# matteo-bastico/MI-Seg

Hardware: AMD Instinct MI355X
Metric: 96^3 patches/sec fwd+bwd, C-Swin-UNETR fs=48 6-class (higher is better)
Workload: dtype bf16; 1 GPU; configs[1]: C-Swin-UNETR feature_size=48 heads=(3,6,12,24) instance_cond, 96^3 patch, 6 classes, batch 1 per GPU, fwd+bwd (+ gradient all-reduce at N>1); global_batch=1

## Files before the change

### include/miseg_hip.h

```cpp
#ifndef MISEG_HIP_H
#define MISEG_HIP_H
#include <stddef.h>
#include <stdint.h>

#ifdef __cplusplus
extern "C" {
#endif

typedef void* miseg_stream_t;

enum { MISEG_F32 = 0, MISEG_BF16 = 1 };
enum { MISEG_OK = 0, MISEG_E_BADARG = -1, MISEG_E_UNSUPPORTED = -2, MISEG_E_LAUNCH = -3 };
enum { MISEG_ACT_NONE = 0, MISEG_ACT_LEAKY = 1, MISEG_ACT_GELU = 2, MISEG_ACT_PRELU = 3 };
#define MISEG_MAX_STYLES 4

#define MISEG_ABI_VERSION 16
int miseg_abi_version(void);
const char* miseg_last_error(void);
int miseg_device_arch(char* buf, size_t n);

size_t miseg_instnorm_stat_bytes(int B, int C);
typedef struct {
  const void* x; int64_t ldx;
  int B, S, C, dtype;
// ... 199 lines not shown
typedef struct {
  const void* qkv; int64_t ldq; void* out; int64_t ldo;
  const float* qkv_bias;
  const float* bias_table;
  float* lse;
  int B, D, H, W, C, heads, dtype;
  int wd, wh, ww, sd, sh, sw, tw;
  float scale;
  float drop_p; uint64_t drop_seed, drop_stream; const uint64_t* drop_step_dev;
} miseg_winattn_params;
int miseg_winattn_fwd(const miseg_winattn_params* p, miseg_stream_t stream);
int miseg_winattn_on_matrix_cores(const miseg_winattn_params* p);

typedef struct {
  miseg_winattn_params f;
  const void* dout; int64_t lddo;
  void* dqkv; int64_t lddq;
  float* dqkv_bias;
  float* dbias_table;
} miseg_winattn_bwd_params;
int miseg_winattn_bwd(const miseg_winattn_bwd_params* p, miseg_stream_t stream);
int miseg_winattn_bwd_on_matrix_cores(const miseg_winattn_bwd_params* p);

typedef struct { const void* a; int64_t lda; const void* b; int64_t ldb; void* y; int64_t ldy; int64_t rows; int C, dtype; } miseg_add_params;
int miseg_add(const miseg_add_params* p, miseg_stream_t stream);
typedef struct { uint32_t struct_size; const void* a; int64_t lda; const void* x; int64_t ldx; void* y; int64_t ldy; const float* coef; int B, S, C, dtype; } miseg_affine2_params;
int miseg_affine2(const miseg_affine2_params* p, miseg_stream_t stream);

typedef struct { const void* src; int64_t lds; int sdtype; void* dst; int64_t ldd; int ddtype; int64_t rows; int C; } miseg_copy2d_params;
int miseg_copy2d(const miseg_copy2d_params* p, miseg_stream_t stream);

typedef struct { const float* src; void* dst; int R, C, dtype, transpose; } miseg_cast_params;
int miseg_cast_matrix(const miseg_cast_params* p, miseg_stream_t stream);

typedef struct {
  const float* src; void* dst;
  int32_t R, C, transpose, inner, outer, tile0;
} miseg_cast_desc;
int miseg_param_cast_batch(const miseg_cast_desc* descs_dev, int ndesc, int total_tiles, int dtype, const int64_t* params_version, int64_t* state,
                           miseg_stream_t stream);

typedef struct { const void* x; int64_t ldx; void* y; int64_t ldy; int64_t rows; int C, dtype; } miseg_gelu_fwd_params;
int miseg_gelu_fwd(const miseg_gelu_fwd_params* p, miseg_stream_t stream);
typedef struct { const void* dy; int64_t lddy; const void* x; int64_t ldx; void* dx; int64_t lddx; int64_t rows; int C, dtype; } miseg_gelu_bwd_params;
int miseg_gelu_bwd(const miseg_gelu_bwd_params* p, miseg_stream_t stream);

// ... 331 lines not shown
```

### mi-seg_amd/csrc/attention.hip

```cpp
#include "common.h"

namespace miseg {

struct WinGeom {
  int B, D, H, W, C, heads, hd;
  int wd, wh, ww, sd, sh, sw, tw;
  int Dp, Hp, Wp, nwd, nwh, nww, n;
  float scale;
};

__device__ __forceinline__ void token_info(const WinGeom& g, int win, int t, int& row, int& label, int& code) {
  int wi = win;
  const int wx = wi % g.nww; wi /= g.nww;
  const int wy = wi % g.nwh; wi /= g.nwh;
  const int wz = wi % g.nwd;
  const int b = wi / g.nwd;
  const int tz = t / (g.wh * g.ww), ty = (t / g.ww) % g.wh, tx = t % g.ww;
  const int pz = wz * g.wd + tz, py = wy * g.wh + ty, px = wx * g.ww + tx;
  int z = pz + g.sd; if (z >= g.Dp) z -= g.Dp;
  int y = py + g.sh; if (y >= g.Hp) y -= g.Hp;
  int x = px + g.sw; if (x >= g.Wp) x -= g.Wp;
  row = (z < g.D && y < g.H && x < g.W) ? ((b * g.D + z) * g.H + y) * g.W + x : -1;
  const int rz = g.sd ? (pz < g.Dp - g.wd ? 0 : (pz < g.Dp - g.sd ? 1 : 2)) : 0;
  const int ry = g.sh ? (py < g.Hp - g.wh ? 0 : (py < g.Hp - g.sh ? 1 : 2)) : 0;
// ... 331 lines not shown
  bf16x8 f;
#pragma unroll
  for (int j = 0; j < 8; ++j) f[j] = (bf16)0.f;
  if (r < 16) {
    const bf16* p = base + r * ATT_VT_LD + t0 + 16 * s + 4 * h;
    const bf16x4 lo = *reinterpret_cast<const bf16x4*>(p);
    const bf16x4 hi = *reinterpret_cast<const bf16x4*>(p + 8);
    f = bf16x8{lo[0], lo[1], lo[2], lo[3], hi[0], hi[1], hi[2], hi[3]};
  }
  return f;
}

__device__ __forceinline__ void att_load16v(const bf16* p, bool vec, float* dst) {
  if (vec) {
    const bf16x8 a = *reinterpret_cast<const bf16x8*>(p), b = *reinterpret_cast<const bf16x8*>(p + 8);
#pragma unroll
    for (int d = 0; d < 8; ++d) { dst[d] = to_f32(a[d]); dst[8 + d] = to_f32(b[d]); }
  } else {
#pragma unroll
    for (int d = 0; d < 16; ++d) dst[d] = to_f32(p[d]);
  }
}

__device__ __forceinline__ void att_unit(int heads, int& win, int& head) {
  const int nb = gridDim.x, xcd = blockIdx.x & 7, q = nb >> 3, r = nb & 7;
  const int unit = xcd * q + (xcd < r ? xcd : r) + (blockIdx.x >> 3);
  win = unit / heads;
  head = unit - win * heads;
}

template <bool MASK, int NW = 4, bool DROP = false>
__global__ void __launch_bounds__(NW * 64) winattn_fwd_mfma_kernel(const bf16* __restrict__ qkv, int64_t ldq, bf16* __restrict__ out, int64_t ldo,
                                                               const float* __restrict__ qkv_bias, const float* __restrict__ bias_table,
                                                               float* __restrict__ lse_out, WinGeom g, int tsize, bool vec, AttnDrop dr) {
  extern __shared__ __attribute__((aligned(16))) char smem[];
  bf16* Qs = reinterpret_cast<bf16*>(smem);
  bf16* Ks = Qs + ATT_NP * 16;
  bf16* Vt = Ks + ATT_NP * 16;
  int* kofs = reinterpret_cast<int*>(Vt + 16 * ATT_VT_LD);
  int* klab = kofs + ATT_NP;
  int* rowq = klab + ATT_NP;
  float* table = reinterpret_cast<float*>(rowq + ATT_NP);
  int win, head;
  att_unit(g.heads, win, head);
  const int tid = threadIdx.x;
  const int n = g.n, C = g.C, ntiles = (n + 31) / 32;
  for (int t = tid; t < ntiles * 32; t += NW * 64) {
    int row = -1, label = 0, code = 0;
    float q[16], k[16], v[16];
#pragma unroll
    for (int d = 0; d < 16; ++d) q[d] = k[d] = v[d] = 0.f;
    if (t < n) {
      token_info(g, win, t, row, label, code);
      if (row >= 0) {
        const bf16* p = qkv + (int64_t)row * ldq + head * 16;
        att_load16v(p, vec, q);
        att_load16v(p + C, vec, k);
        att_load16v(p + 2 * C, vec, v);
      } else if (qkv_bias) {
#pragma unroll
        for (int d = 0; d < 16; ++d) { q[d] = qkv_bias[head * 16 + d]; k[d] = qkv_bias[C + head * 16 + d]; v[d] = qkv_bias[2 * C + head * 16 + d]; }
      }
    }
    const float qs = g.scale * ATT_LOG2E;
#pragma unroll
    for (int d = 0; d < 16; ++d) q[d] *= qs;
    *reinterpret_cast<bf16x8*>(Qs + t * 16) = cvt8(q);
    *reinterpret_cast<bf16x8*>(Qs + t * 16 + 8) = cvt8(q + 8);
    *reinterpret_cast<bf16x8*>(Ks + t * 16) = cvt8(k);
    *reinterpret_cast<bf16x8*>(Ks + t * 16 + 8) = cvt8(k + 8);
#pragma unroll
    for (int d = 0; d < 16; ++d) Vt[d * ATT_VT_LD + t] = (bf16)v[d];
    kofs[t] = code * 4;
    klab[t] = label;
    rowq[t] = row;
  }
  for (int i = tid; i < tsize; i += NW * 64) table[i] = bias_table[(int64_t)i * g.heads + head] * ATT_LOG2E;
  __syncthreads();
  const int lane = tid & 63, wave = __builtin_amdgcn_readfirstlane(tid >> 6), r = lane & 31, h = lane >> 5;
  const int tb = 2 * g.tw - 1;
  const int centre = ((g.tw - 1) * tb + (g.tw - 1)) * tb + (g.tw - 1);
  const bool ragged = (n & 31) != 0;
  constexpr float MASKV = -100.f * ATT_LOG2E;
  const uint64_t dk0 = DROP ? dropout_step_key(dr.key, dr.step_dev) : 0ull;
  const int dcg = (n + 3) / 4;
  for (int qt = wave; qt < ntiles; qt += NW) {
    const int qi = qt * 32 + r;
    const int64_t drow = ((int64_t)win * g.heads + head) * n + qi;
    const bf16x8 qf = *reinterpret_cast<const bf16x8*>(Qs + qi * 16 + 8 * h);
    const char* tq = reinterpret_cast<const char*>(table) + kofs[qi] + 4 * centre;
    const int lq = klab[qi];
    float m = -INFINITY, l = 0.f;
    f32x16 acc;
#pragma unroll
    for (int i = 0; i < 16; ++i) acc[i] = 0.f;
    auto key_tile = [&](int kt, auto last_tag) {
      constexpr bool LAST = decltype(last_tag)::value;
      const bf16x8 kf = *reinterpret_cast<const bf16x8*>(Ks + (kt * 32 + r) * 16 + 8 * h);
      f32x16 sacc;
#pragma unroll
      for (int i = 0; i < 16; ++i) sacc[i] = 0.f;
      sacc = __builtin_amdgcn_mfma_f32_32x32x16_bf16(kf, qf, sacc, 0, 0, 0);
      float sv[16];
#pragma unroll
      for (int gq = 0; gq < 4; ++gq) {
        const int k0 = kt * 32 + 8 * gq + 4 * h;
        const int4 ko = *reinterpret_cast<const int4*>(kofs + k0);
        const int kov[4] = {ko.x, ko.y, ko.z, ko.w};
#pragma unroll
// ... 102 lines not shown

template <bool MASK, bool DT , int NW = 4, bool DROP = false>
__global__ void __launch_bounds__(NW * 64, 2) winattn_bwd_mfma_kernel(const bf16* __restrict__ qkv, int64_t ldq, const bf16* __restrict__ out, int64_t ldo,
                                                                  const bf16* __restrict__ dout, int64_t lddo, bf16* __restrict__ dqkv, int64_t lddq,
                                                                  const float* __restrict__ qkv_bias, const float* __restrict__ bias_table,
                                                                  const float* __restrict__ lse_in, float* __restrict__ dqkv_bias,
                                                                  float* __restrict__ dbias_table, WinGeom g, int tsize, bool vec, AttnDrop dr) {
  extern __shared__ __attribute__((aligned(16))) char smem[];
  constexpr int NI = 24 / NW, NTHR = NW * 64;
  float* table = reinterpret_cast<float*>(smem);
  int* dtable = reinterpret_cast<int*>(table + ATT_TMAX);
  float* padb = reinterpret_cast<float*>(dtable + ATT_TMAX);
  unsigned* bound = reinterpret_cast<unsigned*>(padb + 48);
  char* dstile = reinterpret_cast<char*>(padb + 64);
  float* dqpart = reinterpret_cast<float*>(dstile + NW * 16 * ATT_DS_LD);
  int* qcode = reinterpret_cast<int*>(dqpart + 2 * NW * 256);
  int* qlabel = qcode + ATT_NP;
  int* rowq = qlabel + ATT_NP;
  float* nlse = reinterpret_cast<float*>(rowq + ATT_NP);
  float* ndelta = nlse + ATT_NP;
  bf16* Qs = reinterpret_cast<bf16*>(ndelta + ATT_NP);
  bf16* Gs = Qs + ATT_NP * 16;
  bf16* Ks = Gs + ATT_NP * 16;
  int win, head;
  att_unit(g.heads, win, head);
  const int tid = threadIdx.x;
  const int n = g.n, C = g.C, nt16 = (n + 15) / 16;
  if (tid < 52) padb[tid] = 0.f;
  __syncthreads();
  float mg2 = 0.f, mv2 = 0.f, mda = 0.f;
  for (int t = tid; t < nt16 * 16; t += NTHR) {
    int row = -1, label = 0, code = 0;
    float q[16], k[16], go[16];
    float dl = 0.f, ls = INFINITY, g2 = 0.f, v2 = 0.f;
#pragma unroll
    for (int d = 0; d < 16; ++d) q[d] = k[d] = go[d] = 0.f;
    if (t < n) {
      token_info(g, win, t, row, label, code);
      ls = lse_in[((int64_t)win * g.heads + head) * n + t];
      float v[16];
      if (row >= 0) {
        float o[16];
        att_load16(qkv + (int64_t)row * ldq + head * 16, vec, q);
        att_load16(qkv + (int64_t)row * ldq + C + head * 16, vec, k);
        att_load16(qkv + (int64_t)row * ldq + 2 * C + head * 16, vec, v);
        att_load16(dout + (int64_t)row * lddo + head * 16, vec, go);
        att_load16(out + (int64_t)row * ldo + head * 16, vec, o);
#pragma unroll
// ... 280 lines not shown

static bool fwd_takes_mfma(const miseg_winattn_params* p, const WinGeom& g) {
  return p->dtype == MISEG_BF16 && g.hd == 16 && g.n <= ATT_NP && p->bias_table && ((uintptr_t)p->out % 8 == 0) && p->ldo % 4 == 0;
}

extern "C" int miseg_winattn_on_matrix_cores(const miseg_winattn_params* p) {
  WinGeom g;
  if (!p || make_geom(p, &g)) return 0;
  return (fwd_takes_mfma(p, g) || global_attn_takes(p)) ? 1 : 0;
}

static bool bwd_takes_mfma(const miseg_winattn_bwd_params* p, const WinGeom& g) {
  const int tb = 2 * g.tw - 1;
  return p->f.dtype == MISEG_BF16 && g.hd == 16 && g.n <= ATT_NP && p->f.bias_table && tb * tb * tb <= ATT_TMAX && ((uintptr_t)p->dqkv % 8 == 0) && p->lddq % 4 == 0 &&
         ((uintptr_t)p->f.qkv % 8 == 0) && p->f.ldq % 4 == 0;
}

extern "C" int miseg_winattn_bwd_on_matrix_cores(const miseg_winattn_bwd_params* p) {
  WinGeom g;
  if (!p || !p->dout || !p->dqkv || make_geom(&p->f, &g)) return 0;
  return (bwd_takes_mfma(p, g) || global_attn_bwd_takes(p)) ? 1 : 0;
}

extern "C" int miseg_winattn_fwd(const miseg_winattn_params* p, miseg_stream_t s_) {
  hipStream_t s = (hipStream_t)s_;
  MISEG_REQUIRE(p, MISEG_E_BADARG, "winattn_fwd: null params");
  WinGeom g;
  int rc = make_geom(p, &g);
  if (rc) return rc;
  MISEG_REQUIRE(p->drop_p >= 0.f && p->drop_p < 1.f, MISEG_E_BADARG, "winattn_fwd: drop_p = %f must lie in [0, 1)", (double)p->drop_p);
  const AttnDrop dr = attn_drop_args(p);
  if (global_attn_fwd(p, dr, s, &rc)) return rc;
  const int tb = 2 * g.tw - 1, tsize = p->bias_table ? tb * tb * tb : 0;
  const size_t sh = attn_smem_bytes(g.n, g.hd, tsize, false);
  MISEG_REQUIRE(sh <= 160 * 1024, MISEG_E_UNSUPPORTED, "winattn_fwd: %zu bytes of LDS needed", sh);
  dim3 grid(g.B * g.nwd * g.nwh * g.nww, g.heads);
  const int threads = cdiv(g.n, 64) * 64;
  if (fwd_takes_mfma(p, g)) {
    const size_t shm = attn_mfma_fwd_smem(tsize);
    const bool vec = p->ldq % 8 == 0 && (uintptr_t)p->qkv % 16 == 0;
    const bool wide = (int64_t)grid.x * grid.y < 256;
#define FWD_MFMA_D(M, NWV, D)                                                                                                                  \
  MISEG_SET_SMEM((winattn_fwd_mfma_kernel<M, NWV, D>), shm);                    \
  winattn_fwd_mfma_kernel<M, NWV, D><<<grid.x * grid.y, NWV * 64, shm, s>>>((const bf16*)p->qkv, p->ldq, (bf16*)p->out, p->ldo, p->qkv_bias, p->bias_table, \
                                                                 p->lse, g, tsize, vec, dr)
#define FWD_MFMA(M, NWV) do { if (dr.thresh) { FWD_MFMA_D(M, NWV, true); } else { FWD_MFMA_D(M, NWV, false); } } while (0)
    if ((g.sd | g.sh | g.sw) != 0) { if (wide) { FWD_MFMA(true, 11); } else { FWD_MFMA(true, 8); } }
    else { if (wide) { FWD_MFMA(false, 11); } else { FWD_MFMA(false, 8); } }
#undef FWD_MFMA
#undef FWD_MFMA_D
    MISEG_LAUNCH_CHECK("winattn_fwd_mfma");
    return MISEG_OK;
  }
  return dispatch_dtype(p->dtype, [&](auto* tag) -> int {
    typedef typename std::remove_pointer<decltype(tag)>::type T;
    HD_SWITCH(g.hd / 4, {
      MISEG_SET_SMEM((winattn_fwd_kernel<T, HD4>), sh);
      winattn_fwd_kernel<T, HD4><<<grid, threads, sh, s>>>((const T*)p->qkv, p->ldq, (T*)p->out, p->ldo, p->qkv_bias, p->bias_table, p->lse, g, tsize, dr);
    });
    MISEG_LAUNCH_CHECK("winattn_fwd");
    return MISEG_OK;
  });
}

extern "C" int miseg_winattn_bwd(const miseg_winattn_bwd_params* p, miseg_stream_t s_) {
  hipStream_t s = (hipStream_t)s_;
  MISEG_REQUIRE(p && p->dout && p->dqkv, MISEG_E_BADARG, "winattn_bwd: null pointer");
  MISEG_REQUIRE(!p->dbias_table || p->f.bias_table, MISEG_E_BADARG, "winattn_bwd: dbias_table given without a bias_table");
  WinGeom g;
  int rc = make_geom(&p->f, &g);
  if (rc) return rc;
  MISEG_REQUIRE(p->f.drop_p >= 0.f && p->f.drop_p < 1.f, MISEG_E_BADARG, "winattn_bwd: drop_p = %f must lie in [0, 1)", (double)p->f.drop_p);
  const AttnDrop dr = attn_drop_args(&p->f);
  if (global_attn_bwd(p, dr, s, &rc)) return rc;
  const int tb = 2 * g.tw - 1, tsize = p->f.bias_table ? tb * tb * tb : 0;
  const size_t sh = attn_smem_bytes(g.n, g.hd, tsize, true);
  MISEG_REQUIRE(sh <= 160 * 1024, MISEG_E_UNSUPPORTED, "winattn_bwd: %zu bytes of LDS needed", sh);
  dim3 grid(g.B * g.nwd * g.nwh * g.nww, g.heads);
  const int threads = cdiv(g.n, 64) * 64;
  if (bwd_takes_mfma(p, g)) {
    const bool vec = p->f.ldq % 8 == 0 && p->f.ldo % 8 == 0 && p->lddo % 8 == 0 && (uintptr_t)p->f.qkv % 16 == 0 && (uintptr_t)p->f.out % 16 == 0 &&
                     (uintptr_t)p->dout % 16 == 0;
    const bool wide = true;
    const size_t shm = attn_mfma_bwd_smem(tsize, wide ? 8 : 4);
#define BWD_MFMA_X(M, D, NWV, X)                                                                                                                            \
// ... 28 lines not shown
```

### mi-seg_amd/csrc/common.cpp

```cpp
#include "common.h"
#include "../../include/miseg_hip_debug.h"
#include <string.h>

#ifndef MISEG_COMPILED_ARCH
#define MISEG_COMPILED_ARCH "gfx950"
#endif

namespace miseg {
static thread_local char g_err[512] = "";

int set_error(int code, const char* fmt, ...) {
  va_list ap;
  va_start(ap, fmt);
  vsnprintf(g_err, sizeof(g_err), fmt, ap);
  va_end(ap);
  return code;
}
}

extern "C" int miseg_abi_version(void) { return MISEG_ABI_VERSION; }

extern "C" size_t miseg_abi_struct_size(const char* name) {
  if (!name) return 0;
#define MISEG_SZ(T) if (strcmp(name, #T) == 0) return sizeof(T);
  MISEG_SZ(miseg_instnorm_stats_params) MISEG_SZ(miseg_instnorm_apply_params) MISEG_SZ(miseg_instnorm_bwd_params) MISEG_SZ(miseg_instnorm_pair_bwd_params)
  MISEG_SZ(miseg_layernorm_fwd_params) MISEG_SZ(miseg_layernorm_bwd_params) MISEG_SZ(miseg_gemm_params) MISEG_SZ(miseg_tn_reduce_desc) MISEG_SZ(miseg_gemm_tn_desc) MISEG_SZ(miseg_gemm_tn_stream_desc) MISEG_SZ(miseg_gemm_tn_stream_plan)
  MISEG_SZ(miseg_mlp_params) MISEG_SZ(miseg_colsum_params) MISEG_SZ(miseg_colsum_desc) MISEG_SZ(miseg_conv3_params) MISEG_SZ(miseg_pack_conv3_params) MISEG_SZ(miseg_pack_conv3_desc)
  MISEG_SZ(miseg_conv3_wgrad_params) MISEG_SZ(miseg_conv3_plan_info) MISEG_SZ(miseg_conv3_wgrad_plan_info) MISEG_SZ(miseg_winattn_params) MISEG_SZ(miseg_winattn_bwd_params) MISEG_SZ(miseg_add_params) MISEG_SZ(miseg_copy2d_params)
  MISEG_SZ(miseg_cast_params) MISEG_SZ(miseg_cast_desc) MISEG_SZ(miseg_gelu_fwd_params) MISEG_SZ(miseg_gelu_bwd_params) MISEG_SZ(miseg_s2c_params)
  MISEG_SZ(miseg_patch_embed_params) MISEG_SZ(miseg_patch_embed_bwd_params) MISEG_SZ(miseg_conv3_thin_params) MISEG_SZ(miseg_conv3_thin_wgrad_params)
  MISEG_SZ(miseg_resample2_params) MISEG_SZ(miseg_upsample_cat_params) MISEG_SZ(miseg_upsample_cat_bwd_params) MISEG_SZ(miseg_rowbias_params) MISEG_SZ(miseg_prelu_fwd_params) MISEG_SZ(miseg_prelu_bwd_params) MISEG_SZ(miseg_head_params)
  MISEG_SZ(miseg_head_bwd_params) MISEG_SZ(miseg_im2col3_params) MISEG_SZ(miseg_seg_loss_params) MISEG_SZ(miseg_dice_metric_params) MISEG_SZ(miseg_surface_distance_params) MISEG_SZ(miseg_surface_metrics_params) MISEG_SZ(miseg_surface_dice_params) MISEG_SZ(miseg_opt_desc) MISEG_SZ(miseg_opt_pack_map)
  MISEG_SZ(miseg_opt_step_params) MISEG_SZ(miseg_stitch_params) MISEG_SZ(miseg_aug_sample) MISEG_SZ(miseg_augment_params) MISEG_SZ(miseg_resample3d_params) MISEG_SZ(miseg_label_export_params) MISEG_SZ(miseg_keep_largest_params) MISEG_SZ(miseg_fill_holes_params) MISEG_SZ(miseg_dropout_params)
  MISEG_SZ(miseg_affine2_params) MISEG_SZ(miseg_graph_split_info) MISEG_SZ(miseg_norm_ref) MISEG_SZ(miseg_ensemble_params) MISEG_SZ(miseg_aug_affine_sample) MISEG_SZ(miseg_augment_affine_params)
  MISEG_SZ(miseg_net_end_launch) MISEG_SZ(miseg_head_bwd_plan_info)
#undef MISEG_SZ
  return 0;
}
extern "C" const char* miseg_last_error(void) { return miseg::g_err; }
extern "C" int miseg_device_arch(char* buf, size_t n) {
  if (!buf || n == 0) return MISEG_E_BADARG;
  strncpy(buf, MISEG_COMPILED_ARCH, n);
  buf[n - 1] = 0;
  return MISEG_OK;
}

extern "C" int miseg_device_check(int device) {
  hipDeviceProp_t prop;
  if (hipGetDeviceProperties(&prop, device) != hipSuccess) {
    (void)hipGetLastError();
    return miseg::set_error(MISEG_E_BADARG, "device_check: no HIP device %d", device);
// ... 62 lines not shown
```

### mi-seg_amd/hip/lib.py

```python
import ctypes as C
import os

HERE = os.path.dirname(os.path.abspath(__file__))
LIB_PATH = os.environ.get("MISEG_HIP_LIB") or os.path.join(os.path.dirname(HERE), "csrc", "libmiseg_hip.so")

F32, BF16 = 0, 1
ACT_NONE, ACT_LEAKY, ACT_GELU, ACT_PRELU = 0, 1, 2, 3
MAX_STYLES = 4

vp, i64, i32, f32 = C.c_void_p, C.c_int64, C.c_int, C.c_float
fp4 = vp * MAX_STYLES


class _S(C.Structure):
    pass


ABI_VERSION = 16
C_NAMES = {}


def _struct(name, fields, cname=None):
    t = type(name, (C.Structure,), {"_fields_": fields})
    C_NAMES[t] = cname
# ... 40 lines not shown
                                                                                  ("pad_", i32), ("workspace_bytes", i64)])
TN_STREAM_GROUP_CAP = 8
Colsum = _struct("Colsum", cname="miseg_colsum_params", fields=[("x", vp), ("ldx", i64), ("rows", i64), ("C", i32), ("dtype", i32), ("out", vp), ("accumulate", i32)])
Conv3 = _struct("Conv3", cname="miseg_conv3_params", fields=[("x", vp), ("ldx", i64), ("y", vp), ("ldy", i64), ("wpk", vp), ("B", i32), ("D", i32), ("H", i32),
                          ("W", i32), ("Cin", i32), ("Cout", i32), ("dtype", i32), ("workspace", vp), ("res", vp), ("ldres", i64), ("stat", vp), ("background", i32), ("defer_slabs", i32),
                          ("sc_x", vp), ("ld_sc_x", i64), ("sc_w", vp), ("sc_C", i32), ("s2c_out", vp), ("s2c_C", i32),
                          ("fs_w", vp), ("fs_y", vp), ("ld_fs_y", i64), ("fs_stat", vp)])
PackConv3Desc = _struct("PackConv3Desc", cname="miseg_pack_conv3_desc", fields=[("w", vp), ("fwd_pack", vp), ("bwd_pack", vp), ("Cin", i32), ("Cout", i32), ("tile0", i32), ("pad_", i32)])
PackConv3 = _struct("PackConv3", cname="miseg_pack_conv3_params", fields=[("w", vp), ("fwd_pack", vp), ("bwd_pack", vp), ("Cin", i32), ("Cout", i32), ("dtype", i32)])
Conv3Wgrad = _struct("Conv3Wgrad", cname="miseg_conv3_wgrad_params", fields=[("x", vp), ("ldx", i64), ("dy", vp), ("lddy", i64), ("dw", vp), ("B", i32), ("D", i32),
                                    ("H", i32), ("W", i32), ("Cin", i32), ("Cout", i32), ("dtype", i32), ("accumulate", i32),
                                    ("workspace", vp), ("max_workgroups", i32)])
CONV3_GENERIC, CONV3_FWD96, CONV3_FWD_TINY = 0, 1, 2
Conv3Plan = _struct("Conv3Plan", cname="miseg_conv3_plan_info", fields=[("kernel", i32), ("splits", i32), ("workspace_bytes", C.c_size_t), ("res", i32), ("stat", i32),
                                  ("sc", i32), ("s2c", i32), ("fs", i32), ("defer_slabs", i32)])
CONV3_WGRAD_F32, CONV3_WGRAD_NARROW, CONV3_WGRAD_TINY, CONV3_WGRAD_BF16 = 0, 1, 2, 3
Conv3WgradPlan = _struct("Conv3WgradPlan", cname="miseg_conv3_wgrad_plan_info", fields=[("kernel", i32), ("pad_", i32), ("workspace_bytes", C.c_size_t)])
Winattn = _struct("Winattn", cname="miseg_winattn_params", fields=[("qkv", vp), ("ldq", i64), ("out", vp), ("ldo", i64), ("qkv_bias", vp), ("bias_table", vp),
                              ("lse", vp), ("B", i32), ("D", i32), ("H", i32), ("W", i32), ("C", i32), ("heads", i32),
                              ("dtype", i32), ("wd", i32), ("wh", i32), ("ww", i32), ("sd", i32), ("sh", i32), ("sw", i32),
                              ("tw", i32), ("scale", f32), ("drop_p", f32), ("drop_seed", C.c_uint64), ("drop_stream", C.c_uint64), ("drop_step_dev", vp)])
WinattnBwd = _struct("WinattnBwd", cname="miseg_winattn_bwd_params", fields=[("f", Winattn), ("dout", vp), ("lddo", i64), ("dqkv", vp), ("lddq", i64),
                                    ("dqkv_bias", vp), ("dbias_table", vp)])
Add = _struct("Add", cname="miseg_add_params", fields=[("a", vp), ("lda", i64), ("b", vp), ("ldb", i64), ("y", vp), ("ldy", i64), ("rows", i64), ("C", i32), ("dtype", i32)])
GraphSplitInfo = _struct("GraphSplitInfo", cname="miseg_graph_split_info", fields=[("nodes", i32), ("lanes", i32), ("segments", i32), ("crossing_edges", i32),
                                                                                  ("side_streams", i32), ("main_lane_nodes", i32), ("streams_concurrent", i32)])
Affine2 = _struct("Affine2", cname="miseg_affine2_params", fields=[("struct_size", C.c_uint32), ("a", vp), ("lda", i64), ("x", vp), ("ldx", i64), ("y", vp), ("ldy", i64), ("coef", vp),
                                                                  ("B", i32), ("S", i32), ("C", i32), ("dtype", i32)])
Copy2d = _struct("Copy2d", cname="miseg_copy2d_params", fields=[("src", vp), ("lds", i64), ("sdtype", i32), ("dst", vp), ("ldd", i64), ("ddtype", i32), ("rows", i64), ("C", i32)])
CastDesc = _struct("CastDesc", cname="miseg_cast_desc", fields=[("src", vp), ("dst", vp), ("R", i32), ("C", i32), ("transpose", i32), ("inner", i32), ("outer", i32), ("tile0", i32)])
Resample2 = _struct("Resample2", cname="miseg_resample2_params", fields=[("x", vp), ("ldx", i64), ("y", vp), ("ldy", i64), ("B", i32), ("D", i32), ("H", i32), ("W", i32), ("C", i32),
                                  ("dtype", i32), ("dir", i32)])
UpsampleCat = _struct("UpsampleCat", cname="miseg_upsample_cat_params", fields=[("skip", vp), ("ldskip", i64), ("x", vp), ("ldx", i64), ("out", vp), ("ldout", i64),
                                      ("B", i32), ("D", i32), ("H", i32), ("W", i32), ("Cs", i32), ("Cu", i32), ("factor", i32), ("dtype", i32)])
UpsampleCatBwd = _struct("UpsampleCatBwd", cname="miseg_upsample_cat_bwd_params", fields=[("dcat", vp), ("lddcat", i64), ("dx", vp), ("lddx", i64), ("B", i32), ("D", i32),
                                            ("H", i32), ("W", i32), ("C", i32), ("factor", i32), ("dtype", i32)])
Rowbias = _struct("Rowbias", cname="miseg_rowbias_params", fields=[("x", vp), ("ldx", i64), ("bias", vp), ("y", vp), ("ldy", i64), ("rows", i64), ("C", i32), ("dtype", i32)])
PreluFwd = _struct("PreluFwd", cname="miseg_prelu_fwd_params", fields=[("x", vp), ("ldx", i64), ("slope", vp), ("y", vp), ("ldy", i64), ("rows", i64), ("C", i32), ("dtype", i32)])
PreluBwd = _struct("PreluBwd", cname="miseg_prelu_bwd_params", fields=[("dy", vp), ("lddy", i64), ("x", vp), ("ldx", i64), ("slope", vp), ("dx", vp), ("lddx", i64), ("dslope", vp),
                                ("rows", i64), ("C", i32), ("dtype", i32), ("scratch", vp)])
Cast = _struct("Cast", cname="miseg_cast_params", fields=[("src", vp), ("dst", vp), ("R", i32), ("C", i32), ("dtype", i32), ("transpose", i32)])
GeluFwd = _struct("GeluFwd", cname="miseg_gelu_fwd_params", fields=[("x", vp), ("ldx", i64), ("y", vp), ("ldy", i64), ("rows", i64), ("C", i32), ("dtype", i32)])
GeluBwd = _struct("GeluBwd", cname="miseg_gelu_bwd_params", fields=[("dy", vp), ("lddy", i64), ("x", vp), ("ldx", i64), ("dx", vp), ("lddx", i64), ("rows", i64), ("C", i32), ("dtype", i32)])
S2C = _struct("S2C", cname="miseg_s2c_params", fields=[("src", vp), ("lds", i64), ("dst", vp), ("ldd", i64), ("B", i32), ("D", i32), ("H", i32), ("W", i32),
                      ("C", i32), ("dtype", i32), ("offsets", C.c_int8 * 24)])
PatchEmbed = _struct("PatchEmbed", cname="miseg_patch_embed_params", fields=[("x", vp), ("y", vp), ("ldy", i64), ("w", vp), ("bias", vp), ("B", i32), ("Cin", i32), ("D", i32),
# ... 132 lines not shown
    "miseg_colsum": (i32, [C.POINTER(Colsum), vp]),
    "miseg_gemm_tn_splits": (i32, [C.POINTER(Gemm)]),
    "miseg_gemm_tn_fuses_colsum": (i32, [C.POINTER(Gemm)]),
    "miseg_gemm_tn_reduce_batch": (i32, [vp, i32, vp]),
    "miseg_gemm_tn_group": (i32, [vp, i32, i32, vp]),
    "miseg_gemm_tn_stream_group_plan": (i32, [vp, i32, vp]),
    "miseg_gemm_tn_stream_group": (i32, [vp, i32, vp]),
    "miseg_gemm_tn_stream_group_target": (i32, []),
    "miseg_colsum_batch": (i32, [vp, i32, i32, vp]),
    "miseg_conv3_fwd_plan": (i32, [C.POINTER(Conv3), C.POINTER(Conv3Plan)]),
    "miseg_conv3_fwd": (i32, [C.POINTER(Conv3), vp]),
    "miseg_pack_conv3_elems": (C.c_size_t, [i32, i32, i32, i32]),
    "miseg_pack_conv3_tiles": (i32, [i32, i32, i32]),
    "miseg_pack_conv3_weight": (i32, [C.POINTER(PackConv3), vp]),
    "miseg_pack_conv3_batch": (i32, [vp, i32, i32, i32, vp, vp, vp]),
    "miseg_conv3_wgrad_plan": (i32, [C.POINTER(Conv3Wgrad), C.POINTER(Conv3WgradPlan)]),
    "miseg_conv3_wgrad": (i32, [C.POINTER(Conv3Wgrad), vp]),
    "miseg_conv3_wgrad_group_workspace_bytes": (C.c_size_t, [C.POINTER(Conv3Wgrad), i32]),
    "miseg_conv3_wgrad_group": (i32, [C.POINTER(Conv3Wgrad), i32, vp, vp]),
    "miseg_winattn_fwd": (i32, [C.POINTER(Winattn), vp]),
    "miseg_winattn_on_matrix_cores": (i32, [vp]),
    "miseg_winattn_bwd": (i32, [C.POINTER(WinattnBwd), vp]),
    "miseg_winattn_bwd_on_matrix_cores": (i32, [vp]),
    "miseg_add": (i32, [C.POINTER(Add), vp]),
    "miseg_affine2": (i32, [C.POINTER(Affine2), vp]),
    "miseg_instnorm_bwd_reduce": (i32, [C.POINTER(InstnormBwd), vp]),
    "miseg_copy2d": (i32, [C.POINTER(Copy2d), vp]),
    "miseg_cast_matrix": (i32, [C.POINTER(Cast), vp]),
    "miseg_gelu_fwd": (i32, [C.POINTER(GeluFwd), vp]),
    "miseg_gelu_bwd": (i32, [C.POINTER(GeluBwd), vp]),
    "miseg_space_to_channel": (i32, [C.POINTER(S2C), vp]),
    "miseg_channel_to_space": (i32, [C.POINTER(S2C), vp]),
    "miseg_patch_embed_fwd_plan": (i32, [C.POINTER(PatchEmbed), C.POINTER(NetEndLaunch)]),
    "miseg_patch_embed_fwd": (i32, [C.POINTER(PatchEmbed), vp]),
    "miseg_patch_embed_bwd_workspace_bytes": (C.c_size_t, [C.POINTER(PatchEmbedBwd)]),
    "miseg_patch_embed_bwd_plan": (i32, [C.POINTER(PatchEmbedBwd), C.POINTER(NetEndLaunch)]),
    "miseg_patch_embed_bwd": (i32, [C.POINTER(PatchEmbedBwd), vp]),
    "miseg_conv3_thin_fwd_plan": (i32, [C.POINTER(Conv3Thin), C.POINTER(NetEndLaunch)]),
    "miseg_conv3_thin_fwd": (i32, [C.POINTER(Conv3Thin), vp]),
    "miseg_conv3_thin_wgrad_workspace_bytes": (C.c_size_t, [C.POINTER(Conv3ThinWgrad)]),
    "miseg_conv3_thin_wgrad_plan": (i32, [C.POINTER(Conv3ThinWgrad), C.POINTER(NetEndLaunch)]),
    "miseg_conv3_thin_wgrad": (i32, [C.POINTER(Conv3ThinWgrad), vp]),
    "miseg_head_fwd_plan": (i32, [C.POINTER(Head), C.POINTER(NetEndLaunch)]),
    "miseg_head_fwd": (i32, [C.POINTER(Head), vp]),
    "miseg_head_bwd_plan": (i32, [C.POINTER(HeadBwd), C.POINTER(HeadBwdPlan)]),
    "miseg_head_bwd": (i32, [C.POINTER(HeadBwd), vp]),
# ... 128 lines not shown
```

### mi-seg_amd/hip/ops.py

```python
import ctypes as C
import os
import threading

import torch

from . import lib as L


def _dt(t):
    if t.dtype == torch.float32:
        return L.F32
    if t.dtype == torch.bfloat16:
        return L.BF16
    raise ValueError(f"unsupported dtype {t.dtype} (float32 / bfloat16 only)")


def _stream():
    return C.c_void_p(torch.cuda.current_stream().cuda_stream)


def _ptr(t):
    return C.c_void_p(t.data_ptr()) if t is not None else C.c_void_p(0)


# ... 912 lines not shown
            d.clear()
    check_tn_stream_closed()
    if n:
        raise RuntimeError(f"{n} deferred data-gradient slab sum(s) were never consumed (conv3(..., dx_to_norm=True) in front of something that is no instance norm)")


def check_tn_stream_closed(queues=None):
    for q in ([queues] if queues is not None else _all_queues()):
        n = len(q.tn_stream) + (len(q.side.tn_stream) if q.side is not None else 0)
        if n:
            q.tn_stream.clear()
            if q.side is not None:
                q.side.tn_stream.clear()
            raise RuntimeError(f"{n} streaming weight-gradient product(s) were queued and never launched (tn_stream_close / flush)")


FRESH = 256


def _rows_ptr(t):
    return (FRESH, t[1], t[1], _dt(t[0])) if isinstance(t, tuple) else (_ptr(t), rows(t)[0], t.shape[-1], _dt(t))


def _plan(fn, p, plan):
    L.check(getattr(L.load(), fn)(C.byref(p), C.byref(plan)), fn)
    return plan


def conv3_fwd_plan(x, Cout, **pieces):
    ptr, ld, Cin, dt = _rows_ptr(x)
    p = L.Conv3(ptr, ld, FRESH, Cout, FRESH, *_vol(x[0] if isinstance(x, tuple) else x), Cin, Cout, dt, **pieces)
    return _plan("miseg_conv3_fwd_plan", p, L.Conv3Plan())


def conv3_fuses_shortcut(x, Cout, g, w=None):
    gp, ldg, Csc, gdt = _rows_ptr((x[0] if isinstance(x, tuple) else x, g) if isinstance(g, int) else g)
    if gdt != _rows_ptr(x)[3] or (w is not None and not (w.is_contiguous() and _dt(w) == gdt)):
        return False
    return bool(conv3_fwd_plan(x, Cout, sc_x=gp, ld_sc_x=ldg, sc_w=_ptr(w) if w is not None else FRESH, sc_C=Csc).sc)


def conv3_fuses_s2c(x, Cout, C_left):
    return bool(conv3_fwd_plan(x, Cout, s2c_out=FRESH, s2c_C=C_left).s2c)


def conv3_fuses_fwd_shortcut(x, Cout, w=None):
    if w is not None and not (w.is_contiguous() and w.dtype == x.dtype):
        return False
# ... 249 lines not shown

def im2col3(x, adjoint=False, C_out=None):
    B, D, H, W = _vol(x)
    ld, n, Cc = rows(x)
    if not adjoint:
        out = torch.empty(B, D, H, W, 27 * Cc, dtype=x.dtype, device=x.device)
        _call("miseg_im2col3", L.Im2col3(_ptr(x), ld, _ptr(out), 27 * Cc, B, D, H, W, Cc, _dt(x)))
    else:
        Co = Cc // 27
        out = torch.empty(B, D, H, W, Co, dtype=x.dtype, device=x.device)
        _call("miseg_col2im3", L.Im2col3(_ptr(x), ld, _ptr(out), Co, B, D, H, W, Co, _dt(x)))
    return out


def winattn_params(qkv, out, qkv_bias, table, lse, heads, window, shift, tw, scale, drop=None):
    B, D, H, W = _vol(qkv)
    ldq, n, C3 = rows(qkv)
    Cc = C3 // 3
    dp, (seed, sid, step) = drop if drop else (0.0, (0, 0, None))
    return L.Winattn(_ptr(qkv), ldq, _ptr(out), rows(out)[0], _ptr(qkv_bias), _ptr(table), _ptr(lse), B, D, H, W, Cc, heads, _dt(qkv),
                     window[0], window[1], window[2], shift[0], shift[1], shift[2], tw, scale, float(dp), seed, sid, _ptr(step))


def winattn_fwd(qkv, qkv_bias, table, heads, window, shift, tw, scale, drop=None):
    B, D, H, W = _vol(qkv)
    Cc = qkv.shape[-1] // 3
    out = torch.empty(B, D, H, W, Cc, dtype=qkv.dtype, device=qkv.device)
    nw = B * -(-D // window[0]) * -(-H // window[1]) * -(-W // window[2])
    lse = torch.empty(nw, heads, window[0] * window[1] * window[2], dtype=torch.float32, device=qkv.device)
    n = window[0] * window[1] * window[2]
    _call("miseg_winattn_fwd", winattn_params(qkv, out, qkv_bias, table, lse, heads, window, shift, tw, scale, drop),
          prof=("winattn", 4.0 * nw * heads * n * n * (Cc // heads), _nb(qkv, out, lse)))
    return out, lse


def winattn_bwd(qkv, out, lse, dout, qkv_bias, table, heads, window, shift, tw, scale, dqkv_bias, dtable, drop=None):
    dqkv = torch.empty(qkv.shape, dtype=qkv.dtype, device=qkv.device)
    f = winattn_params(qkv, out, qkv_bias, table, lse, heads, window, shift, tw, scale, drop)
    p = L.WinattnBwd(f, _ptr(dout), rows(dout)[0], _ptr(dqkv), rows(dqkv)[0], _ptr(dqkv_bias), _ptr(dtable))
    B, D, H, W = _vol(qkv)
    n = window[0] * window[1] * window[2]
    nw = B * -(-D // window[0]) * -(-H // window[1]) * -(-W // window[2])
    _call("miseg_winattn_bwd", p, prof=("winattn", 10.0 * nw * heads * n * n * (qkv.shape[-1] // 3 // heads), _nb(qkv, out, lse, dout, dqkv)))
    return dqkv


def add(a, b, out=None):
    lda, n, Cc = rows(a)
    y = out if out is not None else torch.empty(a.shape, dtype=a.dtype, device=a.device)
    _call("miseg_add", L.Add(_ptr(a), lda, _ptr(b), rows(b)[0], _ptr(y), rows(y)[0], n, Cc, _dt(a)))
    return y


def copy2d(src, dst):
    lds, n, Cc = rows(src)
# ... 555 lines not shown
```

Measured before the change: 168.1 patches/s.

## Split tail-round window-attention units across query tiles to fill idle CUs

Adds a planner that, when the number of (window, head) units does not divide evenly by the CU count, splits the leftover units into several workgroups that each handle a range of query tiles. A simple cost model weighs the repeated K/V prologue against the shorter query loop. The Python forward now always plans using the device CU count and calls the new workspace entry point. Split pieces reload K/V and the bias table redundantly, and the cost model constants are heuristic.

Measured after the change: 168.9 patches/s, median of 6. No clear change (+0.5%).

```diff
diff --git a/include/miseg_hip.h b/include/miseg_hip.h
--- a/include/miseg_hip.h
+++ b/include/miseg_hip.h
@@ -245,6 +245,14 @@
 int miseg_winattn_bwd(const miseg_winattn_bwd_params* p, miseg_stream_t stream);
 int miseg_winattn_bwd_on_matrix_cores(const miseg_winattn_bwd_params* p);
 
+typedef struct {
+  int32_t cus;
+  int32_t n_whole, pieces, workgroups;
+  size_t workspace_bytes;
+} miseg_winattn_plan_info;
+int miseg_winattn_plan(const miseg_winattn_params* p, int backward, miseg_winattn_plan_info* plan);
+int miseg_winattn_fwd_ws(const miseg_winattn_params* p, const miseg_winattn_plan_info* force, void* workspace, size_t workspace_bytes, miseg_stream_t stream);
+
 typedef struct { const void* a; int64_t lda; const void* b; int64_t ldb; void* y; int64_t ldy; int64_t rows; int C, dtype; } miseg_add_params;
 int miseg_add(const miseg_add_params* p, miseg_stream_t stream);
 typedef struct { uint32_t struct_size; const void* a; int64_t lda; const void* x; int64_t ldx; void* y; int64_t ldy; const float* coef; int B, S, C, dtype; } miseg_affine2_params;
diff --git a/mi-seg_amd/csrc/attention.hip b/mi-seg_amd/csrc/attention.hip
--- a/mi-seg_amd/csrc/attention.hip
+++ b/mi-seg_amd/csrc/attention.hip
@@ -377,17 +377,33 @@
   }
 }
 
-__device__ __forceinline__ void att_unit(int heads, int& win, int& head) {
-  const int nb = gridDim.x, xcd = blockIdx.x & 7, q = nb >> 3, r = nb & 7;
-  const int unit = xcd * q + (xcd < r ? xcd : r) + (blockIdx.x >> 3);
-  win = unit / heads;
-  head = unit - win * heads;
+struct AttSplit { int n_whole, pieces; };
+struct AttPiece { int win, head, t0, t1, idx , slot ; };
+
+__device__ __forceinline__ AttPiece att_unit(int heads, const AttSplit& sp, int tiles) {
+  AttPiece u;
+  int unit;
+  if ((int)blockIdx.x < sp.n_whole) {
+    const int nb = sp.n_whole, xcd = blockIdx.x & 7, q = nb >> 3, r = nb & 7;
+    unit = xcd * q + (xcd < r ? xcd : r) + (blockIdx.x >> 3);
+    u.t0 = 0; u.t1 = tiles; u.idx = -1; u.slot = 0;
+  } else {
+    const int j = blockIdx.x - sp.n_whole;
+    u.slot = j / sp.pieces;
+    u.idx = j - u.slot * sp.pieces;
+    unit = sp.n_whole + u.slot;
+    u.t0 = u.idx * tiles / sp.pieces;
+    u.t1 = (u.idx + 1) * tiles / sp.pieces;
+  }
+  u.win = unit / heads;
+  u.head = unit - u.win * heads;
+  return u;
 }
 
 template <bool MASK, int NW = 4, bool DROP = false>
 __global__ void __launch_bounds__(NW * 64) winattn_fwd_mfma_kernel(const bf16* __restrict__ qkv, int64_t ldq, bf16* __restrict__ out, int64_t ldo,
                                                                const float* __restrict__ qkv_bias, const float* __restrict__ bias_table,
-                                                               float* __restrict__ lse_out, WinGeom g, int tsize, bool vec, AttnDrop dr) {
+                                                               float* __restrict__ lse_out, WinGeom g, int tsize, bool vec, AttnDrop dr, AttSplit sp) {
   extern __shared__ __attribute__((aligned(16))) char smem[];
   bf16* Qs = reinterpret_cast<bf16*>(smem);
   bf16* Ks = Qs + ATT_NP * 16;
@@ -396,11 +412,12 @@
   int* klab = kofs + ATT_NP;
   int* rowq = klab + ATT_NP;
   float* table = reinterpret_cast<float*>(rowq + ATT_NP);
-  int win, head;
-  att_unit(g.heads, win, head);
+  const int n = g.n, C = g.C, ntiles = (n + 31) / 32;
+  const AttPiece u = att_unit(g.heads, sp, ntiles);
+  const int win = u.win, head = u.head;
   const int tid = threadIdx.x;
-  const int n = g.n, C = g.C, ntiles = (n + 31) / 32;
   for (int t = tid; t < ntiles * 32; t += NW * 64) {
+    const bool own = t >= u.t0 * 32 && t < u.t1 * 32;
     int row = -1, label = 0, code = 0;
     float q[16], k[16], v[16];
 #pragma unroll
@@ -409,7 +426,7 @@
       token_info(g, win, t, row, label, code);
       if (row >= 0) {
         const bf16* p = qkv + (int64_t)row * ldq + head * 16;
-        att_load16v(p, vec, q);
+        if (own) att_load16v(p, vec, q);
         att_load16v(p + C, vec, k);
         att_load16v(p + 2 * C, vec, v);
       } else if (qkv_bias) {
@@ -439,7 +456,7 @@
   constexpr float MASKV = -100.f * ATT_LOG2E;
   const uint64_t dk0 = DROP ? dropout_step_key(dr.key, dr.step_dev) : 0ull;
   const int dcg = (n + 3) / 4;
-  for (int qt = wave; qt < ntiles; qt += NW) {
+  for (int qt = u.t0 + wave; qt < u.t1; qt += NW) {
     const int qi = qt * 32 + r;
     const int64_t drow = ((int64_t)win * g.heads + head) * n + qi;
     const bf16x8 qf = *reinterpret_cast<const bf16x8*>(Qs + qi * 16 + 8 * h);
@@ -588,8 +605,8 @@
   bf16* Qs = reinterpret_cast<bf16*>(ndelta + ATT_NP);
   bf16* Gs = Qs + ATT_NP * 16;
   bf16* Ks = Gs + ATT_NP * 16;
-  int win, head;
-  att_unit(g.heads, win, head);
+  const AttPiece u = att_unit(g.heads, AttSplit{(int)gridDim.x, 1}, 1);
+  const int win = u.win, head = u.head;
   const int tid = threadIdx.x;
   const int n = g.n, C = g.C, nt16 = (n + 15) / 16;
   if (tid < 52) padb[tid] = 0.f;
@@ -916,8 +933,70 @@
   return (bwd_takes_mfma(p, g) || global_attn_bwd_takes(p)) ? 1 : 0;
 }
 
-extern "C" int miseg_winattn_fwd(const miseg_winattn_params* p, miseg_stream_t s_) {
+static constexpr float ATT_FWD_PROLOGUE_SHARE = 0.65f;
+static constexpr float ATT_SPLIT_MIN_GAIN = 0.10f;
+static constexpr float ATT_SPLIT_TIE = 0.002f;
+static constexpr int ATT_MIN_LAST_ROUND = 16;
+
+static int att_fwd_waves(int64_t units) { return units < 256 ? 11 : 8; }
+
+static void att_whole_plan(int units, miseg_winattn_plan_info* pl) {
+  pl->n_whole = units; pl->pieces = 1; pl->workgroups = units; pl->workspace_bytes = 0;
+}
+
+static void att_plan(const WinGeom& g, int units, int cus, miseg_winattn_plan_info* pl) {
+  att_whole_plan(units, pl);
+  const int R = cus > 0 ? cus : 256;
+  const int rem = units % R;
+  if (rem == 0) return;
+  const int tiles = (g.n + 31) / 32;
+  const int pmax = std::min(tiles, R / rem);
+  if (pmax < 2) return;
+  auto steps = [&](int t) { return (t + 3) / 4; };
+  const int whole = steps(tiles);
+  float cost[ATT_MAXT + 1], best = 1.f;
+  for (int pc = 2; pc <= pmax; ++pc) {
+    cost[pc] = ATT_FWD_PROLOGUE_SHARE + (1.f - ATT_FWD_PROLOGUE_SHARE) * (float)steps((tiles + pc - 1) / pc) / (float)whole;
+    best = std::min(best, cost[pc]);
+  }
+  if (best > 1.f - ATT_SPLIT_MIN_GAIN) return;
+  int bp = 1;
+  for (int pc = pmax; pc >= 2; --pc)
+    if (cost[pc] <= best + ATT_SPLIT_TIE && (bp == 1 || units < R || rem * pc >= ATT_MIN_LAST_ROUND)) bp = pc;
+  pl->n_whole = units - rem; pl->pieces = bp; pl->workgroups = pl->n_whole + rem * bp;
+}
+
+static int att_check_plan(const WinGeom& g, int units, const miseg_winattn_plan_info& pl, const char* who) {
+  const int tiles = (g.n + 31) / 32;
+  MISEG_REQUIRE(pl.n_whole >= 0 && pl.n_whole <= units && pl.pieces >= 1 && pl.pieces <= tiles, MISEG_E_BADARG,
+                "%s: plan (n_whole %d, pieces %d) outside %d units of %d query tiles", who, pl.n_whole, pl.pieces, units, tiles);
+  return MISEG_OK;
+}
+
+static int att_device_cus() {
+  static int cus = 0;
+  if (!cus) {
+    int dev = 0, v = 0;
+    if (hipGetDevice(&dev) == hipSuccess && hipDeviceGetAttribute(&v, hipDeviceAttributeMultiprocessorCount, dev) == hipSuccess && v > 0) cus = v;
+    else cus = 256;
+  }
+  return cus;
+}
+
+extern "C" int miseg_winattn_plan(const miseg_winattn_params* p, int backward, miseg_winattn_plan_info* plan) {
+  MISEG_REQUIRE(p && plan, MISEG_E_BADARG, "winattn_plan: null pointer");
+  WinGeom g;
+  if (const int rc = make_geom(p, &g)) return rc;
+  const int cus = plan->cus;
+  const int units = g.B * g.nwd * g.nwh * g.nww * g.heads;
+  if (!backward && fwd_takes_mfma(p, g)) att_plan(g, units, cus, plan); else att_whole_plan(units, plan);
+  plan->cus = cus;
+  return MISEG_OK;
+}
+
+static int winattn_fwd_impl(const miseg_winattn_params* p, const miseg_winattn_plan_info* force, bool planned, void* ws, size_t wsb, miseg_stream_t s_) {
   hipStream_t s = (hipStream_t)s_;
+  (void)ws; (void)wsb;
   MISEG_REQUIRE(p, MISEG_E_BADARG, "winattn_fwd: null params");
   WinGeom g;
   int rc = make_geom(p, &g);
@@ -933,11 +1012,19 @@
   if (fwd_takes_mfma(p, g)) {
     const size_t shm = attn_mfma_fwd_smem(tsize);
     const bool vec = p->ldq % 8 == 0 && (uintptr_t)p->qkv % 16 == 0;
-    const bool wide = (int64_t)grid.x * grid.y < 256;
+    const int units = (int)(grid.x * grid.y);
+    const bool wide = att_fwd_waves(units) == 11;
+    miseg_winattn_plan_info pl;
+    if (force) pl = *force;
+    else if (planned) att_plan(g, units, att_device_cus(), &pl);
+    else att_whole_plan(units, &pl);
+    if (const int prc = att_check_plan(g, units, pl, "winattn_fwd")) return prc;
+    const AttSplit sp{pl.n_whole, pl.pieces};
+    const int nwg = pl.n_whole + (units - pl.n_whole) * pl.pieces;
 #define FWD_MFMA_D(M, NWV, D)                                                                                                                  \
   MISEG_SET_SMEM((winattn_fwd_mfma_kernel<M, NWV, D>), shm);                    \
-  winattn_fwd_mfma_kernel<M, NWV, D><<<grid.x * grid.y, NWV * 64, shm, s>>>((const bf16*)p->qkv, p->ldq, (bf16*)p->out, p->ldo, p->qkv_bias, p->bias_table, \
-                                                                 p->lse, g, tsize, vec, dr)
+  winattn_fwd_mfma_kernel<M, NWV, D><<<nwg, NWV * 64, shm, s>>>((const bf16*)p->qkv, p->ldq, (bf16*)p->out, p->ldo, p->qkv_bias, p->bias_table, \
+                                                                 p->lse, g, tsize, vec, dr, sp)
 #define FWD_MFMA(M, NWV) do { if (dr.thresh) { FWD_MFMA_D(M, NWV, true); } else { FWD_MFMA_D(M, NWV, false); } } while (0)
     if ((g.sd | g.sh | g.sw) != 0) { if (wide) { FWD_MFMA(true, 11); } else { FWD_MFMA(true, 8); } }
     else { if (wide) { FWD_MFMA(false, 11); } else { FWD_MFMA(false, 8); } }
@@ -946,6 +1033,7 @@
     MISEG_LAUNCH_CHECK("winattn_fwd_mfma");
     return MISEG_OK;
   }
+  MISEG_REQUIRE(!force || force->pieces <= 1, MISEG_E_UNSUPPORTED, "winattn_fwd: only the bf16 head_dim-16 matrix-core kernel splits its units");
   return dispatch_dtype(p->dtype, [&](auto* tag) -> int {
     typedef typename std::remove_pointer<decltype(tag)>::type T;
     HD_SWITCH(g.hd / 4, {
@@ -955,6 +1043,12 @@
     MISEG_LAUNCH_CHECK("winattn_fwd");
     return MISEG_OK;
   });
+}
+
+extern "C" int miseg_winattn_fwd(const miseg_winattn_params* p, miseg_stream_t s) { return winattn_fwd_impl(p, nullptr, false, nullptr, 0, s); }
+
+extern "C" int miseg_winattn_fwd_ws(const miseg_winattn_params* p, const miseg_winattn_plan_info* force, void* workspace, size_t workspace_bytes, miseg_stream_t s) {
+  return winattn_fwd_impl(p, force, true, workspace, workspace_bytes, s);
 }
 
 extern "C" int miseg_winattn_bwd(const miseg_winattn_bwd_params* p, miseg_stream_t s_) {
diff --git a/mi-seg_amd/csrc/common.cpp b/mi-seg_amd/csrc/common.cpp
--- a/mi-seg_amd/csrc/common.cpp
+++ b/mi-seg_amd/csrc/common.cpp
@@ -26,7 +26,7 @@
   MISEG_SZ(miseg_instnorm_stats_params) MISEG_SZ(miseg_instnorm_apply_params) MISEG_SZ(miseg_instnorm_bwd_params) MISEG_SZ(miseg_instnorm_pair_bwd_params)
   MISEG_SZ(miseg_layernorm_fwd_params) MISEG_SZ(miseg_layernorm_bwd_params) MISEG_SZ(miseg_gemm_params) MISEG_SZ(miseg_tn_reduce_desc) MISEG_SZ(miseg_gemm_tn_desc) MISEG_SZ(miseg_gemm_tn_stream_desc) MISEG_SZ(miseg_gemm_tn_stream_plan)
   MISEG_SZ(miseg_mlp_params) MISEG_SZ(miseg_colsum_params) MISEG_SZ(miseg_colsum_desc) MISEG_SZ(miseg_conv3_params) MISEG_SZ(miseg_pack_conv3_params) MISEG_SZ(miseg_pack_conv3_desc)
-  MISEG_SZ(miseg_conv3_wgrad_params) MISEG_SZ(miseg_conv3_plan_info) MISEG_SZ(miseg_conv3_wgrad_plan_info) MISEG_SZ(miseg_winattn_params) MISEG_SZ(miseg_winattn_bwd_params) MISEG_SZ(miseg_add_params) MISEG_SZ(miseg_copy2d_params)
+  MISEG_SZ(miseg_conv3_wgrad_params) MISEG_SZ(miseg_conv3_plan_info) MISEG_SZ(miseg_conv3_wgrad_plan_info) MISEG_SZ(miseg_winattn_params) MISEG_SZ(miseg_winattn_bwd_params) MISEG_SZ(miseg_winattn_plan_info) MISEG_SZ(miseg_add_params) MISEG_SZ(miseg_copy2d_params)
   MISEG_SZ(miseg_cast_params) MISEG_SZ(miseg_cast_desc) MISEG_SZ(miseg_gelu_fwd_params) MISEG_SZ(miseg_gelu_bwd_params) MISEG_SZ(miseg_s2c_params)
   MISEG_SZ(miseg_patch_embed_params) MISEG_SZ(miseg_patch_embed_bwd_params) MISEG_SZ(miseg_conv3_thin_params) MISEG_SZ(miseg_conv3_thin_wgrad_params)
   MISEG_SZ(miseg_resample2_params) MISEG_SZ(miseg_upsample_cat_params) MISEG_SZ(miseg_upsample_cat_bwd_params) MISEG_SZ(miseg_rowbias_params) MISEG_SZ(miseg_prelu_fwd_params) MISEG_SZ(miseg_prelu_bwd_params) MISEG_SZ(miseg_head_params)
diff --git a/mi-seg_amd/hip/lib.py b/mi-seg_amd/hip/lib.py
--- a/mi-seg_amd/hip/lib.py
+++ b/mi-seg_amd/hip/lib.py
@@ -86,6 +86,7 @@
                               ("tw", i32), ("scale", f32), ("drop_p", f32), ("drop_seed", C.c_uint64), ("drop_stream", C.c_uint64), ("drop_step_dev", vp)])
 WinattnBwd = _struct("WinattnBwd", cname="miseg_winattn_bwd_params", fields=[("f", Winattn), ("dout", vp), ("lddo", i64), ("dqkv", vp), ("lddq", i64),
                                     ("dqkv_bias", vp), ("dbias_table", vp)])
+WinattnPlan = _struct("WinattnPlan", cname="miseg_winattn_plan_info", fields=[("cus", i32), ("n_whole", i32), ("pieces", i32), ("workgroups", i32), ("workspace_bytes", C.c_size_t)])
 Add = _struct("Add", cname="miseg_add_params", fields=[("a", vp), ("lda", i64), ("b", vp), ("ldb", i64), ("y", vp), ("ldy", i64), ("rows", i64), ("C", i32), ("dtype", i32)])
 GraphSplitInfo = _struct("GraphSplitInfo", cname="miseg_graph_split_info", fields=[("nodes", i32), ("lanes", i32), ("segments", i32), ("crossing_edges", i32),
                                                                                   ("side_streams", i32), ("main_lane_nodes", i32), ("streams_concurrent", i32)])
@@ -264,6 +265,8 @@
     "miseg_winattn_on_matrix_cores": (i32, [vp]),
     "miseg_winattn_bwd": (i32, [C.POINTER(WinattnBwd), vp]),
     "miseg_winattn_bwd_on_matrix_cores": (i32, [vp]),
+    "miseg_winattn_plan": (i32, [C.POINTER(Winattn), i32, C.POINTER(WinattnPlan)]),
+    "miseg_winattn_fwd_ws": (i32, [C.POINTER(Winattn), C.POINTER(WinattnPlan), vp, C.c_size_t, vp]),
     "miseg_add": (i32, [C.POINTER(Add), vp]),
     "miseg_affine2": (i32, [C.POINTER(Affine2), vp]),
     "miseg_instnorm_bwd_reduce": (i32, [C.POINTER(InstnormBwd), vp]),
diff --git a/mi-seg_amd/hip/ops.py b/mi-seg_amd/hip/ops.py
--- a/mi-seg_amd/hip/ops.py
+++ b/mi-seg_amd/hip/ops.py
@@ -958,8 +958,8 @@
     return (FRESH, t[1], t[1], _dt(t[0])) if isinstance(t, tuple) else (_ptr(t), rows(t)[0], t.shape[-1], _dt(t))
 
 
-def _plan(fn, p, plan):
-    L.check(getattr(L.load(), fn)(C.byref(p), C.byref(plan)), fn)
+def _plan(fn, p, plan, *mid):
+    L.check(getattr(L.load(), fn)(C.byref(p), *mid, C.byref(plan)), fn)
     return plan
 
 
@@ -1255,15 +1255,31 @@
                      window[0], window[1], window[2], shift[0], shift[1], shift[2], tw, scale, float(dp), seed, sid, _ptr(step))
 
 
-def winattn_fwd(qkv, qkv_bias, table, heads, window, shift, tw, scale, drop=None):
+_CUS = {}
+
+
+def _cus(device):
+    i = device.index if device.index is not None else torch.cuda.current_device()
+    if i not in _CUS:
+        _CUS[i] = torch.cuda.get_device_properties(i).multi_processor_count
+    return _CUS[i]
+
+
+def winattn_plan(params, backward, cus=256):
+    return _plan("miseg_winattn_plan", params, L.WinattnPlan(cus=cus), int(bool(backward)))
+
+
+def winattn_fwd(qkv, qkv_bias, table, heads, window, shift, tw, scale, drop=None, plan=None):
     B, D, H, W = _vol(qkv)
     Cc = qkv.shape[-1] // 3
     out = torch.empty(B, D, H, W, Cc, dtype=qkv.dtype, device=qkv.device)
     nw = B * -(-D // window[0]) * -(-H // window[1]) * -(-W // window[2])
     lse = torch.empty(nw, heads, window[0] * window[1] * window[2], dtype=torch.float32, device=qkv.device)
     n = window[0] * window[1] * window[2]
-    _call("miseg_winattn_fwd", winattn_params(qkv, out, qkv_bias, table, lse, heads, window, shift, tw, scale, drop),
-          prof=("winattn", 4.0 * nw * heads * n * n * (Cc // heads), _nb(qkv, out, lse)))
+    p = winattn_params(qkv, out, qkv_bias, table, lse, heads, window, shift, tw, scale, drop)
+    if plan is None:
+        plan = winattn_plan(p, False, _cus(qkv.device))
+    _call("miseg_winattn_fwd_ws", p, prof=("winattn", 4.0 * nw * heads * n * n * (Cc // heads), _nb(qkv, out, lse)), extra=(C.byref(plan), None, 0))
     return out, lse
 
 
```
